# pierrebarbera/epa-ng

Hardware: AMD Instinct MI355X
Metric: query placements/sec (whole node), 512-tip GTR+G4 DNA ref, preplace+thorough (higher is better)
Workload: dtype f64; 1 GPU; cfg2: 512-tip DNA GTR+G4 ref, W=1500, 150 bp reads, dyn-heur 0.99999, preplace+thorough; branches=1021, parallelism=query-shard x1 (weak)

## Files before the change

### epa_ng_amd/csrc/epa_dev.hip

```cpp
#include "epa_dev_internal.hpp"

#include <math.h>
#include <string.h>

#include <algorithm>
#include <numeric>
#include <atomic>
#include <thread>

static thread_local std::string g_create_err;

int epa_fail(epa_ctx* ctx, int code, const std::string& msg) {
  if (ctx) ctx->err = msg; else g_create_err = msg;
  return code;
}

namespace {
__global__ void __launch_bounds__(256) k_zero(uint4* __restrict__ a, size_t na, uint4* __restrict__ b, size_t nb) {
  const size_t stride = (size_t)gridDim.x * 256, i0 = (size_t)blockIdx.x * 256 + threadIdx.x;
  const uint4 z = make_uint4(0u, 0u, 0u, 0u);
  for (size_t i = i0; i < na; i += stride) a[i] = z;
  for (size_t i = i0; i < nb; i += stride) b[i] = z;
}
}
// ... 473 lines not shown
}

double log_sum_exp(const double* v, uint32_t K) {
  double mx = v[0], sum = 0.0;
  for (uint32_t j = 1; j < K; ++j) mx = std::max(mx, v[j]);
  for (uint32_t j = 0; j < K; ++j) sum += std::exp(v[j] - mx);
  return mx + std::log(sum);
}
}

extern "C" int epa_quadrature_legendre01(uint32_t K, double* nodes, double* log_weights) {
  if (K < 1 || K > 64 || !nodes || !log_weights) return EPA_ERR_INVALID_ARG;
  std::vector<double> d(K, 0.0), o(K > 1 ? K - 1 : 0), x;
  for (uint32_t i = 1; i < K; ++i) o[i - 1] = (double)i / std::sqrt(4.0 * i * i - 1.0);
  tridiag_eigenvalues(d, o, x);
  for (uint32_t j = 0; j < K; ++j) {
    double t = x[j], dp = 1.0;
    for (int it = 0; it < 3; ++it) {
      double p0 = 1.0, p1 = t;
      for (uint32_t n = 1; n < K; ++n) { const double p2 = ((2.0 * n + 1.0) * t * p1 - n * p0) / (n + 1.0); p0 = p1; p1 = p2; }
      dp = K * (t * p1 - p0) / (t * t - 1.0);
      if (it < 2) t -= p1 / dp;
    }
    nodes[j] = 0.5 * (1.0 + t);
    log_weights[j] = -std::log((1.0 - t) * (1.0 + t)) - 2.0 * std::log(std::fabs(dp));
  }
  const double norm = log_sum_exp(log_weights, K);
  for (uint32_t j = 0; j < K; ++j) log_weights[j] -= norm;
  return EPA_OK;
}

extern "C" int epa_quadrature_laguerre(uint32_t K, double* nodes, double* log_weights) {
  if (K < 1 || K > 64 || !nodes || !log_weights) return EPA_ERR_INVALID_ARG;
  std::vector<double> d(K), o(K > 1 ? K - 1 : 0), x;
  for (uint32_t i = 0; i < K; ++i) d[i] = 2.0 * i + 1.0;
  for (uint32_t i = 1; i < K; ++i) o[i - 1] = (double)i;
  tridiag_eigenvalues(d, o, x);
  for (uint32_t j = 0; j < K; ++j) {
    double t = x[j], lm = 1.0;
    for (int it = 0; it < 3; ++it) {
      double l0 = 1.0, l1 = 1.0 - t;
      for (uint32_t n = 1; n < K; ++n) { const double l2 = ((2.0 * n + 1.0 - t) * l1 - n * l0) / (n + 1.0); l0 = l1; l1 = l2; }
      lm = l0;
      if (it < 2) t -= l1 * t / (K * (l1 - l0));
    }
    nodes[j] = t;
    log_weights[j] = std::log(t) - 2.0 * std::log((double)K) - 2.0 * std::log(std::fabs(lm));
  }
  const double norm = log_sum_exp(log_weights, K);
  for (uint32_t j = 0; j < K; ++j) log_weights[j] -= norm;
  return EPA_OK;
}

extern "C" int epa_dev_device_count(void) {
  int n = 0;
  if (hipGetDeviceCount(&n) != hipSuccess) { (void)hipGetLastError(); return 0; }
  return n;
}

extern "C" const char* epa_dev_last_error(const epa_ctx* ctx) {
  return ctx ? ctx->err.c_str() : g_create_err.c_str();
}

extern "C" int epa_dev_set_query_layout(epa_ctx* ctx, uint32_t code_stride) {
  if (!ctx) return EPA_ERR_INVALID_ARG;
  ctx->code_stride = code_stride;
  return EPA_OK;
}

extern "C" int epa_dev_set_option(epa_ctx* ctx, const char* key, int value) {
  if (!ctx || !key) return EPA_ERR_INVALID_ARG;
  if (strcmp(key, "lookup_block") == 0) {
    if (!ctx->lookup_blocks) return epa_fail(ctx, EPA_ERR_INVALID_ARG, "set_option: lookup_block needs a context in the blocked lookup layout");
    if (value <= 0 || (value & 63)) return epa_fail(ctx, EPA_ERR_INVALID_ARG, "set_option: lookup_block must be a positive multiple of 64");
    for (void* p : ctx->blk_buf)
      if (p) return epa_fail(ctx, EPA_ERR_INVALID_ARG, "set_option: lookup_block must be set before the first preplacement");
    ctx->lookup_block = (uint32_t)value;
    return EPA_OK;
  }
  const bool dedup_key = strcmp(key, "dedup_key_bits") == 0;
  if (dedup_key || strcmp(key, "dedup_sort_bits") == 0) {
    if (value < 0 || value > 64) return epa_fail(ctx, EPA_ERR_INVALID_ARG, std::string("set_option: ") + key + " must be 0 .. 64");
    (dedup_key ? ctx->opt.dedup_key_bits : ctx->opt.dedup_sort_bits) = value;
    return EPA_OK;
  }
  struct Entry { const char* name; int EpaOptions::*field; };
  static const Entry table[] = {
      {"thorough_generic", &EpaOptions::thorough_generic}, {"preplace_generic", &EpaOptions::preplace_generic},
      {"select_full_rows", &EpaOptions::select_full_rows}, {"select_sort", &EpaOptions::select_sort},
      {"queued_thorough", &EpaOptions::queued_thorough},   {"xcd_balance", &EpaOptions::xcd_balance},
      {"aa_valu", &EpaOptions::aa_valu},                   {"timers", &EpaOptions::timers},
      {"newton_lds", &EpaOptions::newton_lds},             {"tip_distal", &EpaOptions::tip_distal},
      {"preplace_screen", &EpaOptions::preplace_screen},   {"preplace_screen_scale", &EpaOptions::preplace_screen_scale}};
  for (const Entry& e : table)
    if (strcmp(key, e.name) == 0) {
      ctx->opt.*e.field = value;
      ctx->generic_thorough = ctx->generic_native || ctx->opt.thorough_generic != 0;
      return EPA_OK;
    }
  return epa_fail(ctx, EPA_ERR_INVALID_ARG, std::string("set_option: unknown key '") + key + "'");
}

extern "C" int epa_dev_set_heuristic(epa_ctx* ctx, int mode, double param) {
  if (!ctx) return EPA_ERR_INVALID_ARG;
  if (mode < EPA_HEUR_DYNAMIC || mode > EPA_HEUR_BASEBALL)
    return epa_fail(ctx, EPA_ERR_INVALID_ARG, "set_heuristic: unknown mode");
  if (mode == EPA_HEUR_FIXED && !(param >= 0.0 && param <= 1.0))
    return epa_fail(ctx, EPA_ERR_INVALID_ARG, "set_heuristic: the fraction must lie in [0, 1]");
  ctx->heur_mode = mode;
  ctx->heur_param = param;
  return EPA_OK;
}

extern "C" int epa_dev_set_query_packing(epa_ctx* ctx, int bits) {
  if (!ctx) return EPA_ERR_INVALID_ARG;
  if (bits != 8 && bits != 4) return epa_fail(ctx, EPA_ERR_INVALID_ARG, "set_query_packing: 8 or 4 bits per code");
  if (bits == 4 && ctx->s != 4)
    return epa_fail(ctx, EPA_ERR_UNSUPPORTED, "set_query_packing: the 4-bit format holds nucleotide codes only");
  ctx->code_packed4 = bits == 4;
  return EPA_OK;
}

extern "C" int epa_pack_codes_4bit(const uint8_t* codes, uint32_t Q, uint32_t stride, uint8_t* packed) {
  if (!codes || !packed) return EPA_ERR_INVALID_ARG;
  const size_t ps = ((size_t)stride + 1) / 2;
  const unsigned cap = g_encode_threads.load(std::memory_order_relaxed);
  const unsigned hw = cap ? cap : std::max(1u, std::thread::hardware_concurrency());
  const unsigned nt = (unsigned)std::min<uint64_t>(std::min(hw, 32u), std::max<uint64_t>(1, (uint64_t)Q * stride >> 20));
  std::vector<int> bad(nt, 0);
  auto work = [&](unsigned t) {
    const uint32_t q0 = (uint32_t)((uint64_t)Q * t / nt), q1 = (uint32_t)((uint64_t)Q * (t + 1) / nt);
    unsigned over = 0;
    for (uint32_t q = q0; q < q1; ++q) {
      const uint8_t* r = codes + (size_t)q * stride;
      uint8_t* o = packed + (size_t)q * ps;
      for (uint32_t p = 0; p < stride / 2; ++p) {
        const uint8_t hi = r[2 * p], lo = r[2 * p + 1];
        over |= hi | lo;
        o[p] = (uint8_t)((hi << 4) | lo);
      }
      if (stride & 1) { const uint8_t hi = r[stride - 1]; over |= hi; o[ps - 1] = (uint8_t)(hi << 4); }
    }
    bad[t] = over > 15;
  };
  if (nt == 1) work(0);
  else {
    std::vector<std::thread> th;
    for (unsigned t = 0; t < nt; ++t) th.emplace_back(work, t);
    for (auto& x : th) x.join();
  }
  for (unsigned t = 0; t < nt; ++t) if (bad[t]) return EPA_ERR_INVALID_ARG;
  return EPA_OK;
}

extern "C" int epa_unpack_codes_4bit(const uint8_t* packed, uint32_t Q, uint32_t stride, uint8_t* codes) {
  if (!codes || !packed) return EPA_ERR_INVALID_ARG;
  const size_t ps = ((size_t)stride + 1) / 2;
  for (uint32_t q = 0; q < Q; ++q)
    for (uint32_t i = 0; i < stride; ++i) {
      const uint8_t b = packed[(size_t)q * ps + i / 2];
      codes[(size_t)q * stride + i] = (i & 1) ? (b & 15u) : (b >> 4);
    }
  return EPA_OK;
}

extern "C" int epa_dev_set_stream(epa_ctx* ctx, void* s) {
// ... 1557 lines not shown
```

### epa_ng_amd/csrc/epa_dev_internal.hpp

```cpp
#pragma once

#include <hip/hip_runtime.h>
#include <stdint.h>

#include <algorithm>
#include <cmath>
#include <string>
#include <vector>

#include <rocprim/device/device_radix_sort.hpp>

#include "epa_dev.h"

using epa_radix_cfg = rocprim::radix_sort_config<rocprim::default_config, rocprim::default_config,
                                                 rocprim::default_config, 0>;

#define EPA_MAX_STATES 20
#define EPA_MAX_CATS 16
#define EPA_MAX_COLS 24
#define EPA_GRID_Y 65535u

struct ModelDNA {
  double U[16];
  double Ui[16];
// ... 135 lines not shown
  uint64_t n = 0;
  SlotState state = SlotState::Free;
  bool unfinished() const { return state == SlotState::Begun || state == SlotState::Launched || state == SlotState::GroupMember; }
  ChunkInputs staged_inputs() const {
    if (x_codes) return {x_codes, x_begin, x_span};
    const char* d = (const char*)d_in;
    const uint32_t* b = (const uint32_t*)(d + codes_bytes);
    return {(const uint8_t*)d, b, b + Q};
  }
  SelectPending sel;
  uint32_t* h_sel = nullptr;
  const uint8_t* l_codes = nullptr;
  const uint32_t *l_begin = nullptr, *l_span = nullptr;
  epa_pair* l_pairs = nullptr;
  epa_result* l_res = nullptr;
  uint32_t l_max_span = 0, l_flags = 0;
  int leader = -1;
  int g_index = 0;
  int g_n = 0;
  int g_left = 0;
  int g_slots[EPA_MAX_GROUP] = {};
  uint32_t g_qoff[EPA_MAX_GROUP + 1] = {};
  uint32_t own_Q = 0;
  const uint8_t* own_x_codes = nullptr;
  const uint32_t *own_x_begin = nullptr, *own_x_span = nullptr;
  void* d_merge = nullptr;
  size_t d_merge_sz = 0;
  epa_pair* d_gpairs = nullptr;
  epa_result* d_gres = nullptr;
  size_t g_cap = 0;
  uint32_t* d_goff = nullptr;
  uint32_t* h_goff = nullptr;

  void lead_merged(uint32_t total, const uint8_t* codes, const uint32_t* begin, const uint32_t* span) {
    own_Q = Q; own_x_codes = x_codes; own_x_begin = x_begin; own_x_span = x_span;
    Q = total; x_codes = codes; x_begin = begin; x_span = span;
  }
  void restore_own() { Q = own_Q; x_codes = own_x_codes; x_begin = own_x_begin; x_span = own_x_span; }
  void group_begun(ChunkSlot* all, const int* slots, int n, const uint32_t* qoff) {
    g_n = n;
    for (int i = 0; i <= n; ++i) g_qoff[i] = qoff[i];
    for (int i = 0; i < n; ++i) {
      g_slots[i] = slots[i];
      all[slots[i]].leader = slots[0];
      all[slots[i]].g_index = i;
      if (i) all[slots[i]].state = SlotState::GroupMember;
    }
  }
  void group_launched(ChunkSlot* all) {
    restore_own();
    g_left = g_n;
    for (int i = 1; i < g_n; ++i) {
      all[g_slots[i]].state = SlotState::Launched;
      all[g_slots[i]].l_flags = l_flags;
    }
  }
  void launch_over(ChunkSlot* all, SlotState to) {
    state = to;
    if (g_n <= 1) return;
    restore_own();
    for (int i = 0; i < g_n; ++i) {
      all[g_slots[i]].leader = -1;
      if (i) all[g_slots[i]].state = to;
    }
    g_n = 0;
    g_left = 0;
  }
};

struct EpaOptions {
  int thorough_generic = 0;
  int preplace_generic = 0;
  int select_full_rows = 0;
  int select_sort = 0;
  int queued_thorough = 0;
  int xcd_balance = 1;
  int aa_valu = 0;
  int timers = 1;
  int newton_lds = 0;
  int tip_distal = 1;
  int dedup_key_bits = 64;
  int preplace_screen = 1;
  int preplace_screen_scale = 1;
  int dedup_sort_bits = 32;
};

struct epa_ctx {
  int device = 0;
  EpaOptions opt;
  int n_cu = 256;
  hipStream_t stream = nullptr;
  std::string err;

  int s = 0, c = 0, ncols = 0;
  int c_in = 0;
  uint32_t W = 0, B = 0;
  ModelDev hmodel;
  ModelDev* dmodel = nullptr;
  ModelDNA dna;
  bool dna_zero0 = false;
  bool rate_scalers = false;
  bool generic_thorough = false;
  bool generic_native = false;
  BloConsts blo;
  int aa_x_as_n = 0;
  uint32_t code_stride = 0;

  double* refT = nullptr;
  uint32_t* scSum = nullptr;
  double* blen = nullptr;
  double* lookup = nullptr;
  double* refI = nullptr;
  uint8_t* resc0 = nullptr;
  double* cinv = nullptr;
  double inv_w0 = 0.0;
  double* lookup2 = nullptr;
  float2* lookup2f = nullptr;
  bool lookup2f_refused = false;
  uint64_t screen_runs = 0;
  double screen_M = 0.0;
  uint64_t screen_nonfinite = 0;
  uint32_t* tip_row = nullptr;
  uint8_t* tipmask = nullptr;
  double* tipd = nullptr;
  bool lookup_built = false;
  double* prof_tab = nullptr;
  bool lookup_blocks = false;
  uint32_t lookup_block = 1024;
  std::vector<double> h_blen;

  static constexpr int N_SCRATCH = 26;
  static constexpr int N_SLOTS = 24;
  static constexpr int N_BANKS = 1 + N_SLOTS;
  int bank = 0;
  void* scratch[N_BANKS * N_SCRATCH] = {};
  size_t scratch_sz[N_BANKS * N_SCRATCH] = {};

  uint32_t select_cap = 64;
  uint32_t* th_ctr = nullptr;
  bool code_packed4 = false;
  int heur_mode = 0;
  double heur_param = 0.0;

  hipStream_t copy_stream = nullptr, down_stream = nullptr;
  ChunkSlot slots[N_SLOTS];

  enum { T_PREPLACE = 0, T_THOROUGH = 1, T_SELECT = 2, T_SCORE = 3, T_SITES = 4, T_RELL = 5, T_MARGINAL = 6, T_RELL_TESTS = 7, T_RELL_AU = 8, T_RELL_KH = 9, T_PREPLACE_PROFILE = 10, T_DEDUP = 11, N_TIMERS = 12 };
  EvTimer t_lookup;
  std::vector<hipEvent_t> blk_ev[N_BANKS];
  uint32_t blk_ev_n[N_BANKS] = {};
  void* blk_buf[N_BANKS] = {};
  size_t blk_sz[N_BANKS] = {};
  EvTimer t_bank[N_BANKS][N_TIMERS];
  uint32_t xcd_cum[9] = {0u, 1u << 17, 2u << 17, 3u << 17, 4u << 17, 5u << 17, 6u << 17, 7u << 17, 1u << 20};
  double xcd_w[8] = {0.125, 0.125, 0.125, 0.125, 0.125, 0.125, 0.125, 0.125};
  double last_sclk_mhz = 0.0;
  bool xstamp_ok = false;
  hipEvent_t ev_rb[N_BANKS] = {};
  hipStream_t side_stream[N_BANKS] = {};
  hipEvent_t ev_fork[N_BANKS] = {}, ev_join[N_BANKS] = {};
  const void* clean_stats[N_BANKS] = {};
  bool clean_ctr[N_BANKS] = {};
  int t_last[N_TIMERS] = {};
  epa_thorough_stats last_stats{};
};

// ... 180 lines not shown
```

### epa_ng_amd/csrc/preplace.hip

```cpp
#include "epa_dev_internal.hpp"
#include "wave_util.hpp"

#include <cstdlib>
#include <cstring>

#include <algorithm>

namespace {

constexpr int GQ = 256;
constexpr int CH = 160;
constexpr int SPREAD = 96;
constexpr int TROWS = CH + SPREAD;
constexpr int NB = 16;
constexpr int CW = CH / 4;

struct Group {
  uint32_t start;
  uint32_t count;
  uint32_t min_begin;
  uint32_t cls;
};

__device__ __forceinline__ void validate_window(uint32_t i, uint32_t begin, uint32_t span, uint32_t W,
// ... 466 lines not shown
#define PP_XCD 1
#endif
using epa_wave::seg_key;
struct SegTrack {
  double m = -INFINITY;
  __device__ __forceinline__ void add(unsigned long long* __restrict__ segmax, uint32_t segp, uint32_t qi, uint32_t b,
                                      bool last, double v) {
    m = fmax(m, v);
    if ((b & 63u) == 63u || last) {
      atomicMax(&segmax[(size_t)qi * segp + (b >> 6)], seg_key(m));
      m = -INFINITY;
    }
  }
};

#ifndef PP_PRIO
#define PP_PRIO 1
#endif
template <int NBATCH>
__device__ __forceinline__ void gather_prio(int bt) {
#if PP_PRIO == 1
  if (bt == 0) __builtin_amdgcn_s_setprio(3);
  else if (bt == NBATCH / 4) __builtin_amdgcn_s_setprio(2);
  else if (bt == NBATCH / 2) __builtin_amdgcn_s_setprio(1);
  else if (bt == (3 * NBATCH) / 4) __builtin_amdgcn_s_setprio(0);
#elif PP_PRIO == 2
  if (bt == 0) __builtin_amdgcn_s_setprio(3);
  else if (bt == NBATCH / 2) __builtin_amdgcn_s_setprio(0);
#elif PP_PRIO == 3
  if (bt == 0) __builtin_amdgcn_s_setprio(3);
  else if (bt == (2 * NBATCH) / 5) __builtin_amdgcn_s_setprio(2);
  else if (bt == (7 * NBATCH) / 10) __builtin_amdgcn_s_setprio(1);
  else if (bt == (9 * NBATCH) / 10) __builtin_amdgcn_s_setprio(0);
#elif PP_PRIO == 4
  if (bt == 0) __builtin_amdgcn_s_setprio(3);
  else if (bt == NBATCH / 10) __builtin_amdgcn_s_setprio(2);
  else if (bt == (3 * NBATCH) / 10) __builtin_amdgcn_s_setprio(1);
  else if (bt == (6 * NBATCH) / 10) __builtin_amdgcn_s_setprio(0);
#endif
}

struct ItemWalk { uint32_t pos, end, step, lo; };
__device__ __forceinline__ ItemWalk item_walk(uint32_t total) {
  if (PP_XCD && (gridDim.x & 7u) == 0) {
    const uint32_t x = blockIdx.x & 7u, local = blockIdx.x >> 3;
    const uint32_t lo = (uint32_t)((uint64_t)total * x / 8), hi = (uint32_t)((uint64_t)total * (x + 1) / 8);
    return {lo + local, hi, gridDim.x >> 3, lo};
  }
  return {blockIdx.x, total, gridDim.x, 0u};
}

#ifndef PP_XCD_GROUPS
#define PP_XCD_GROUPS 1
#endif
__device__ __forceinline__ void item_group_tile(uint32_t v, uint32_t lo, uint32_t hi, uint32_t ng, uint32_t ntiles,
                                                uint32_t& grp, uint32_t& tile) {
  if (!PP_XCD_GROUPS) { grp = v % ng; tile = v / ng; return; }
  const uint32_t gl = lo / ntiles, tl = lo - gl * ntiles, gh = (hi - 1) / ntiles, th = (hi - 1) - gh * ntiles;
  uint32_t r = v - lo;
  for (uint32_t t = 0; t < ntiles; ++t) {
    const uint32_t first = gl + (t < tl ? 1u : 0u), last1 = gh + 1u - (t > th ? 1u : 0u);
    const uint32_t c = last1 > first ? last1 - first : 0u;
    if (r < c) { grp = first + r; tile = t; return; }
    r -= c;
  }
  grp = 0; tile = ntiles;
}

__device__ __forceinline__ uint32_t choose_tile(uint32_t ng, uint32_t B, uint32_t nwg) {
  uint32_t best = 32, best_cost = 0xffffffffu;
  for (uint32_t n = 16; n <= 96; n += 8) {
    const uint32_t items = ng * ((B + n - 1) / n);
    const uint32_t cost = ((items + nwg - 1) / nwg) * (n + 3);
    if (cost <= best_cost) { best_cost = cost; best = n; }
  }
  return best;
}

#ifdef PP_SCHED_PIN
#define PP_SCHED_BARRIER() __builtin_amdgcn_sched_barrier(0)
#else
#define PP_SCHED_BARRIER()
#endif
template <bool ACC, int SPR, int ROWL, bool SPARSE = false>
__global__ void __launch_bounds__(GQ2, 4) k_preplace_pairs(
    const double* __restrict__ lookup2, const uint16_t* __restrict__ packed,
    const uint16_t* __restrict__ tails, const uint32_t* __restrict__ win_begin,
    const uint32_t* __restrict__ win_span, const uint32_t* __restrict__ perm,
    const Group* __restrict__ groups, uint32_t W, uint32_t B, uint32_t pitch, uint32_t NP16,
    const uint32_t* __restrict__ status, double* __restrict__ lnl,
    unsigned long long* __restrict__ segmax, uint32_t segp) {
  constexpr int TR2 = (CH + SPR) / 2;
  extern __shared__ __attribute__((aligned(16))) char smem[];
  static_assert(ROWL % 16 == 0 && ROWL >= PROWB && ((TR2 - 1) * ROWL + PROWB) < 65536, "16-bit LDS offsets");
  double* accs = reinterpret_cast<double*>(smem + (size_t)TR2 * ROWL);
  __shared__ uint32_t s_maxspan;
  __shared__ uint32_t s_qi[GQ2];
  constexpr uint32_t BSTR = GQ2 + 4;
  const uint32_t ng = status[5];
  const uint32_t NBP = SPARSE ? 64u : ACC ? NB2_ACC : choose_tile(ng, B, gridDim.x);
  const uint32_t ntiles = SPARSE ? 1u : (B + NBP - 1) / NBP;
  const int t = threadIdx.x;
  const ItemWalk iw = SPARSE ? ItemWalk{blockIdx.x, ng, gridDim.x, 0u} : item_walk(ng * ntiles);
  for (uint32_t item = iw.pos; item < iw.end; item += iw.step) {
  uint32_t item_g = item, item_t = 0;
  if (!SPARSE) item_group_tile(item, iw.lo, iw.end, ng, ntiles, item_g, item_t);
  const Group g = groups[item_g];
  const uint32_t b0 = SPARSE ? min(g.min_begin * 64u, B - 1u) : item_t * NBP;
  const uint32_t nb = min(NBP, B - b0);
  __syncthreads();
  if (g.count == 0) continue;
  const bool active = t < (int)g.count;
  uint32_t qi = 0, begin = 0, span = 0;
  if (active) {
    qi = perm[g.start + t];
    begin = win_begin[qi];
    span = win_span[qi];
    if ((uint64_t)begin + span > W) span = 0;
  }
  if (t == 0) s_maxspan = 0;
  const uint32_t my_q = (active && span > 0) ? qi : 0xffffffffu;
  s_qi[t] = my_q;
  __syncthreads();
  {
    uint32_t m = span;
#pragma unroll
    for (int off = 32; off; off >>= 1) m = max(m, (uint32_t)__shfl_xor((int)m, off));
    if ((t & 63) == 0) atomicMax(&s_maxspan, m);
  }
  if (ACC) for (uint32_t j = 0; j < nb; ++j) accs[j * GQ2 + t] = 0.0;
  __syncthreads();
  const uint32_t gmin = win_begin[perm[g.start]];
  const uint32_t gspread = win_begin[perm[g.start + g.count - 1]] - gmin;
  const uint32_t rowoff = ((begin - gmin) >> 1) * ROWL;
  const uint32_t rowoff2 = rowoff | (rowoff << 16);
  const uint32_t nchunks = ACC ? (s_maxspan + CH - 1) / CH : 1;
  uint32_t t0 = 0, t1 = 0, t2 = 0, tailchunk = 0xffffffffu;
  if (active && (span & 3)) {
    const uint16_t* tq = tails + (size_t)qi * 4;
    t0 = tq[0] + rowoff; t1 = tq[1] + rowoff; t2 = tq[2] + rowoff;
    tailchunk = ((span >> 2) * 2) / CP;
  }
  auto at = [&](uint32_t off) -> double { return *reinterpret_cast<const double*>(smem + off); };
  SegTrack seg;

  for (uint32_t c = 0; c < nchunks; ++c) {
    const uint32_t cbase = c * CH;
    const bool mine = active && cbase < span;
    uint32_t cw[PW];
    if (mine) {
      const uint4* p = reinterpret_cast<const uint4*>(packed + (size_t)qi * NP16 + (size_t)c * CP);
#pragma unroll
      for (int i = 0; i < PW / 4; ++i) {
        const uint4 v = p[i];
        cw[4 * i] = v.x + rowoff2;
        cw[4 * i + 1] = v.y + rowoff2;
        cw[4 * i + 2] = v.z + rowoff2;
        cw[4 * i + 3] = v.w + rowoff2;
      }
    } else {
#pragma unroll
      for (int i = 0; i < PW; ++i) cw[i] = 0;
    }
    const uint32_t row0 = gmin + cbase;
    const uint32_t need = min((uint32_t)TR2, (gspread >> 1) + (min((uint32_t)CH, s_maxspan - cbase) + 1) / 2);
    const uint32_t rows = (row0 < W) ? min(need, (W - row0 + 1) / 2) : 0;
    const uint32_t n2 = rows * (PE / 2);
    constexpr int PF = (TR2 * (PE / 2) + GQ2 - 1) / GQ2;
    auto request = [&](uint32_t j, double2 (&pfs)[PF]) {
      const double2* src = reinterpret_cast<const double2*>(
          lookup2 + (((size_t)(b0 + j) * 2 + (row0 & 1u)) * ((W + 1) / 2) + (row0 >> 1)) * PE);
#pragma unroll
      for (int u = 0; u < PF; ++u) {
        const uint32_t i = u * GQ2 + t;
        pfs[u] = make_double2(0.0, 0.0);
        if (i < n2) pfs[u] = src[i];
      }
    };
    auto stage = [&](const double2 (&pfs)[PF], uint32_t boff) {
#pragma unroll
      for (int u = 0; u < PF; ++u) {
        const uint32_t i = u * GQ2 + t;
        if (i < n2) {
          if (ROWL == PROWB) {
            reinterpret_cast<double2*>(smem + boff)[i] = pfs[u];
          } else {
            const uint32_t r = i / (PE / 2), c2 = i - r * (PE / 2);
            *reinterpret_cast<double2*>(smem + boff + r * ROWL + c2 * 16) = pfs[u];
          }
        }
      }
    };
    auto gather = [&](uint32_t j, uint32_t boff) {
      if (mine) {
        double sum = ACC ? accs[j * GQ2 + t] : 0.0;
#pragma unroll
        for (int i = 0; i < PW; ++i) asm volatile("" : "+v"(cw[i]));
#ifndef PP_WPB
#define PP_WPB 2
#endif
        constexpr int WPB = PP_WPB, NBATCH = PW / WPB;
        double rb[2][WPB * 2];
        auto issue = [&](int bt) {
#pragma unroll
          for (int w = 0; w < WPB; ++w) {
            const uint32_t v = cw[bt * WPB + w];
            rb[bt & 1][2 * w] = at((v & 0xffffu) + boff);
            rb[bt & 1][2 * w + 1] = at((v >> 16) + boff);
          }
        };
        issue(0);
        PP_SCHED_BARRIER();
#pragma unroll
        for (int bt = 0; bt < NBATCH; ++bt) {
          gather_prio<NBATCH>(bt);
          if (bt + 1 < NBATCH) issue(bt + 1);
          PP_SCHED_BARRIER();
#pragma unroll
          for (int w = 0; w < WPB; ++w) {
            const double s1 = rb[bt & 1][2 * w] + rb[bt & 1][2 * w + 1];
            sum += s1;
          }
          PP_SCHED_BARRIER();
        }
        if (c == tailchunk) {
          sum += at(t0 + boff);
          sum += at(t1 + boff);
          sum += at(t2 + boff);
        }
        if (ACC) {
          accs[j * GQ2 + t] = sum;
        } else {
          accs[(j & 7u) * BSTR + t] = sum;
          if (segmax) seg.add(segmax, segp, qi, b0 + j, j + 1 == nb, sum);
        }
      }
    };
    auto emit_burst = [&](uint32_t kb) {
      __builtin_amdgcn_wave_barrier();
      const uint32_t lane = (uint32_t)t & 63u, wbase = (uint32_t)t & ~63u, c4 = lane & 3u;
      const uint32_t ncol = min(8u, nb - 8u * kb), bcol = b0 + 8u * kb + 2u * c4;
      const uint32_t r0 = 2u * c4, r1 = 2u * c4 + 1u;
#pragma unroll
      for (uint32_t k = 0; k < 4; ++k) {
        const uint32_t tq = wbase + k * 16 + (lane >> 2);
        const uint32_t q = s_qi[tq];
        if (q != 0xffffffffu && 2u * c4 < ncol) {
          const double a0 = accs[r0 * BSTR + tq];
          double* dst = lnl + (size_t)q * pitch + bcol;
          if (2u * c4 + 1u < ncol) *reinterpret_cast<double2*>(dst) = make_double2(a0, accs[r1 * BSTR + tq]);
          else *dst = a0;
        }
      }
      __builtin_amdgcn_wave_barrier();
    };
    auto flush = [&](uint32_t j) {
      if (ACC) return;
      if ((j & 7u) == 7u) emit_burst(j >> 3);
      else if (j + 1 == nb) emit_burst(j >> 3);
    };
    {
      double2 pf[PF];
      request(0, pf);
      for (uint32_t j = 0; j < nb; ++j) {
        __syncthreads();
        stage(pf, 0);
        __syncthreads();
        if (j + 1 < nb) request(j + 1, pf);
        PP_SCHED_BARRIER();
        gather(j, 0);
        flush(j);
// ... 548 lines not shown
  const uint32_t K = pairs ? n_blocks * Wp : sites ? ctx->W + 1 : 0;
  size_t temp_bytes = 0;
  (void)rocprim::radix_sort_pairs<epa_radix_cfg>(nullptr, temp_bytes, (uint32_t*)nullptr, (uint32_t*)nullptr,
                                  (uint32_t*)nullptr, (uint32_t*)nullptr, Q, 0, 32, ctx->stream);
  uint32_t *status, *key_cnt, *iota, *sorted_keys, *perm, *keys;
  const uint32_t nseg = (ctx->B + 63) / 64, seg32p = (nseg + 7u) & ~7u;
  const uint32_t KB = 2 * Wp, n_blocks_c = 2 * nseg;
  const uint64_t max_cells = (uint64_t)Q * nseg;
  const uint32_t Kc = nseg * KB + 1;
  const uint32_t max_runs_c = (uint32_t)std::min<uint64_t>((max_cells + GQ2 - 1) / GQ2 + n_blocks_c, 0xffffffu);
  const uint32_t max_groups_c = max_runs_c + n_blocks_c * n_buckets;
  const size_t smem_c = sizeof(uint32_t) * (2 * (n_blocks_c + 1) + 4 * (size_t)max_runs_c + 2);
  double delta = -1.0;
  constexpr uint64_t SCREEN_MIN_CELLS = 80000000ull;
  const bool big = ctx->opt.preplace_screen >= 2 || probe || (uint64_t)Q * ctx->B >= SCREEN_MIN_CELLS;
  if (pairs && !blocked && nseg <= 64 && max_span != 0 && max_span <= (uint32_t)CH && ctx->opt.preplace_screen && big &&
      (probe || (segmax && t.band_t > 0.0)) && max_cells < 0x80000000ull && smem_c <= 65536) {
    const int brc = launch_build_lookup2f(ctx);
    if (brc) return brc;
    delta = epa_screen_delta(ctx, span_bound);
  }
  const bool screen = delta >= 0.0;
  uint32_t *seg32, *cstatus, *ccnt, *crank, *csorted, *cperm;
  unsigned long long *seg_mask, *n_incl;
  Group* cgroups;
  Group* groups;
  uint16_t *packed, *tails;
  void* temp;
  auto layout = [&](Carver c) {
    status = c.take<uint32_t>(64);
    key_cnt = c.take<uint32_t>(K);
    seg32 = c.take<uint32_t>(screen ? (size_t)Q * seg32p : 0);
    n_incl = c.take<unsigned long long>(screen ? 1 : 0);
    cstatus = c.take<uint32_t>(screen ? 64 : 0);
    ccnt = c.take<uint32_t>(screen ? Kc : 0);
    iota = c.take<uint32_t>(Q);
    sorted_keys = c.take<uint32_t>(Q);
    perm = c.take<uint32_t>(Q);
    keys = c.take<uint32_t>(Q);
    groups = c.take<Group>(max_groups);
    packed = c.take<uint16_t>((size_t)Q * NP16);
    tails = c.take<uint16_t>((pairs || sites) ? 4 * (size_t)Q : 0);
    seg_mask = c.take<unsigned long long>(screen ? Q : 0);
    crank = c.take<uint32_t>(screen ? (size_t)Q * seg32p : 0);
    csorted = c.take<uint32_t>(screen ? max_cells : 0);
    cperm = c.take<uint32_t>(screen ? max_cells : 0);
    cgroups = c.take<Group>(screen ? max_groups_c : 0);
    temp = c.tail(temp_bytes);
    return c.off;
  };
  char* base = (char*)epa_scratch(ctx, SLOT_PREPLACE, layout(Carver{}));
  if (!base) return epa_fail(ctx, EPA_ERR_HIP, "hipMalloc(preplace scratch)");
  layout(Carver{base});
  *d_status = status;
  {
    const int zr = epa_zero_async(ctx, status, (char*)iota - (char*)status, segmax, sizeof(unsigned long long) * (size_t)Q * segp);
    if (zr) return zr;
  }
  const bool acc = max_span == 0 || max_span > (uint32_t)CH;
  const bool wide = pairs && !acc && (uint64_t)Q * SPREAD < (uint64_t)1400 * ctx->W;
  const uint32_t rowl = (wide || acc) ? ROWL_PACKED : ROWL_NARROW;
  if (pairs) {
    constexpr uint32_t pack_grid = 64;
    hipLaunchKernelGGL(k_pack_pairs, dim3(std::min<uint32_t>((Q + 15) / 16, (uint32_t)ctx->n_cu * pack_grid)), dim3(256), 0, ctx->stream, d_codes, d_begin,
                       d_span, Q, ctx->W, cstride, crel, span_bound, Wp, NP16, rowl, packed, tails, keys, K, status);
  } else if (sites) {
    hipLaunchKernelGGL(k_pack_sites<24>, dim3((Q + 3) / 4), dim3(256), 0, ctx->stream, d_codes, d_begin,
                       d_span, Q, ctx->W, cstride, crel, span_bound, NP16, packed, tails, keys, K, status);
  }
  if (pairs || sites) {
    hipLaunchKernelGGL(k_count_keys, dim3((Q + 255) / 256), dim3(256), 0, ctx->stream, keys, Q, key_cnt, iota);
    launch_scan_counts(ctx, key_cnt, K);
    hipLaunchKernelGGL(k_scatter_sorted, dim3((Q + 255) / 256), dim3(256), 0, ctx->stream, keys, iota, key_cnt, Q,
                       sorted_keys, perm);
  } else {
    hipLaunchKernelGGL(k_iota, dim3((Q + 255) / 256), dim3(256), 0, ctx->stream, iota, Q);
    hipLaunchKernelGGL(k_validate, dim3((Q + 255) / 256), dim3(256), 0, ctx->stream, d_begin, d_span, Q,
                       ctx->W, std::min(span_bound, crel ? cstride : 0xffffffffu), status);
    int wbits = 1;
    while (wbits < 32 && (1ull << wbits) <= (uint64_t)ctx->W) ++wbits;
    EPA_HIP(ctx, rocprim::radix_sort_pairs<epa_radix_cfg>(temp, temp_bytes, d_begin, sorted_keys, iota, perm, Q, 0, wbits,
                                           ctx->stream));
  }
  constexpr int SPREAD_WIDE = 288;
  hipLaunchKernelGGL(k_make_groups, dim3(1), dim3(256),
                     sizeof(uint32_t) * (2 * (n_blocks + 1) + 4 * (size_t)max_runs + 2), ctx->stream,
                     sorted_keys, Q, pairs ? Wp : 0xffffffffu, n_blocks, class_blocks, gq0, gq1,
                     (uint32_t)(wide ? SPREAD_WIDE : SPREAD), max_runs, groups, max_groups, status);
  const size_t codes_bytes = (size_t)Q * cstride;
  const uint32_t want_cls = pairs ? 1u : 0u;
  const size_t lds = sizeof(double) * ((size_t)TROWS * ctx->ncols + (acc ? (size_t)NB * GQ : 0));
  const size_t lds2 = wide ? (size_t)((CH + SPREAD_WIDE) / 2) * ROWL_PACKED + sizeof(double) * NB2_BURST * (GQ2 + 4)
                           : (size_t)TROWS2 * rowl + sizeof(double) * (acc ? NB2_ACC * GQ2 : NB2_BURST * (GQ2 + 4));
  const bool acc_s = max_span == 0 || max_span > (uint32_t)CHS;
  const size_t lds_s = (size_t)TROWS_S * 24 * 8 + sizeof(double) * (acc_s ? NB2_ACC_S * GQ2 : NB2_BURST * (GQ2 + 4));
  using FastKernel = decltype(&k_preplace_sites<24, false>);
  using GenericKernel = decltype(&k_preplace<16, false>);
  FastKernel k_fast = nullptr;
  if (pairs) k_fast = wide ? k_preplace_pairs<false, SPREAD_WIDE, ROWL_PACKED> : acc ? k_preplace_pairs<true, SPREAD, ROWL_PACKED> : k_preplace_pairs<false, SPREAD, ROWL_NARROW>;
  else if (sites) k_fast = acc_s ? k_preplace_sites<24, true> : k_preplace_sites<24, false>;
  const bool fast_acc = pairs ? acc : acc_s;
  const size_t lds_fast = pairs ? lds2 : lds_s;
  const GenericKernel k_generic = sites ? nullptr : ctx->ncols == 16 ? (acc ? k_preplace<16, true> : k_preplace<16, false>) : (acc ? k_preplace<24, true> : k_preplace<24, false>);
  if (k_fast) EPA_HIP(ctx, hipFuncSetAttribute((const void*)k_fast, hipFuncAttributeMaxDynamicSharedMemorySize, (int)lds_fast));
  if (k_generic) EPA_HIP(ctx, hipFuncSetAttribute((const void*)k_generic, hipFuncAttributeMaxDynamicSharedMemorySize, (int)lds));
  auto kernels = [&](const double* lk, const double* lk2, uint32_t nB, double* lnl, unsigned long long* sm, bool fast = true) {
    if (k_fast && fast) {
      const uint32_t tile = fast_acc ? (pairs ? NB2_ACC : NB2_ACC_S) : 16;
      const dim3 grid_f((uint32_t)std::min<uint64_t>((uint64_t)max_groups * ((nB + tile - 1) / tile), (uint64_t)ctx->n_cu));
      hipLaunchKernelGGL(k_fast, grid_f, dim3(GQ2), (uint32_t)lds_fast, ctx->stream, pairs ? lk2 : lk, (const uint16_t*)packed,
                         (const uint16_t*)tails, d_begin, d_span, perm, groups, ctx->W, nB, pitch, NP16, status, lnl,
                         fast_acc ? nullptr : sm, segp);
    }
    if (!k_generic) return;
    const uint32_t ntiles = (nB + NB - 1) / NB;
    const dim3 grid(pairs ? (uint32_t)std::min<uint64_t>((uint64_t)max_groups * ntiles, (uint64_t)ctx->n_cu * (acc ? 2 : 4))
                          : max_groups * ntiles);
    hipLaunchKernelGGL(k_generic, grid, dim3(GQ), (uint32_t)lds, ctx->stream, lk, d_codes, d_begin, d_span, perm, groups, ctx->W,
                       cstride, crel, nB, pitch, codes_bytes, want_cls, status, lnl);
  };
  if (probe) probe->ran = screen;
  if (probe && !screen) return EPA_OK;
  if (screen) {
    using ScreenKernel = decltype(&k_preplace_screen<SPREAD, ROWL_NARROW>);
    const ScreenKernel k_screen = wide ? k_preplace_screen<SPREAD_WIDE, ROWL_PACKED> : k_preplace_screen<SPREAD, ROWL_NARROW>;
    const FastKernel k_exact = wide ? k_preplace_pairs<false, SPREAD_WIDE, ROWL_PACKED, true> : k_preplace_pairs<false, SPREAD, ROWL_NARROW, true>;
    const size_t lds_scr = wide ? (size_t)((CH + SPREAD_WIDE) / 2) * ROWL_PACKED : (size_t)TROWS2 * ROWL_NARROW;
    EPA_HIP(ctx, hipFuncSetAttribute((const void*)k_screen, hipFuncAttributeMaxDynamicSharedMemorySize, (int)lds_scr));
    EPA_HIP(ctx, hipFuncSetAttribute((const void*)k_exact, hipFuncAttributeMaxDynamicSharedMemorySize, (int)lds_fast));
    const uint32_t BP = (ctx->B + 1) / 2;
    struct Events {
      hipEvent_t e[3] = {nullptr, nullptr, nullptr};
      ~Events() { for (hipEvent_t x : e) if (x) (void)hipEventDestroy(x); }
    } evs;
    hipEvent_t* const ev = evs.e;
    if (probe) for (hipEvent_t& e : evs.e) EPA_HIP(ctx, hipEventCreate(&e));
    if (probe) EPA_HIP(ctx, hipEventRecord(ev[0], ctx->stream));
    else epa_timer_start(ctx, epa_t(ctx, epa_ctx::T_PREPLACE));
    const dim3 grid_s((uint32_t)std::min<uint64_t>((uint64_t)max_groups * ((BP + 15) / 16), (uint64_t)ctx->n_cu));
    hipLaunchKernelGGL(k_screen, grid_s, dim3(GQ2), (uint32_t)lds_scr, ctx->stream, (const float2*)ctx->lookup2f, (const uint16_t*)packed,
                       (const uint16_t*)tails, d_begin, d_span, perm, groups, ctx->W, BP, NP16, status, seg32, seg32p);
    if (probe) EPA_HIP(ctx, hipEventRecord(ev[1], ctx->stream));
    const double band = (probe ? probe->band_t : t.band_t) + 2.0 * delta;
    hipLaunchKernelGGL(k_screen_band, dim3((Q + 255) / 256), dim3(256), 0, ctx->stream, (const uint32_t*)seg32, Q, nseg, seg32p, band,
                       delta, (const uint32_t*)keys, KB, probe ? nullptr : segmax, segp, probe ? nullptr : ccnt, crank, seg_mask, n_incl);
    if (probe) {
      EPA_HIP(ctx, hipEventRecord(ev[2], ctx->stream));
      EPA_HIP(ctx, hipGetLastError());
      EPA_HIP(ctx, hipEventSynchronize(ev[2]));
      (void)hipEventElapsedTime(&probe->ms_screen, ev[0], ev[1]);
      (void)hipEventElapsedTime(&probe->ms_band, ev[1], ev[2]);
      probe->delta = delta;
      probe->seg32 = seg32;
      probe->mask = seg_mask;
      probe->n_incl = n_incl;
      return EPA_OK;
    }
    ++ctx->screen_runs;
    launch_scan_counts(ctx, ccnt, Kc);
    hipLaunchKernelGGL(k_scatter_cells, dim3((Q + 255) / 256), dim3(256), 0, ctx->stream, (const unsigned long long*)seg_mask,
                       (const uint32_t*)keys, (const uint32_t*)crank, (const uint32_t*)ccnt, Q, seg32p, KB, (uint32_t)max_cells, csorted, cperm);
    hipLaunchKernelGGL(k_make_groups, dim3(1), dim3(256), smem_c, ctx->stream, (const uint32_t*)csorted, (uint32_t)max_cells, Wp, n_blocks_c,
                       n_blocks_c, (uint32_t)GQ2, (uint32_t)GQ2, (uint32_t)(wide ? SPREAD_WIDE : SPREAD), max_runs_c, cgroups, max_groups_c,
                       cstatus, (const uint32_t*)(ccnt + (Kc - 1)), KB);
    hipLaunchKernelGGL(k_exact, dim3(std::min<uint32_t>(max_groups_c, (uint32_t)ctx->n_cu)), dim3(GQ2), (uint32_t)lds_fast, ctx->stream,
                       (const double*)ctx->lookup2, (const uint16_t*)packed, (const uint16_t*)tails, d_begin, d_span, (const uint32_t*)cperm,
                       (const Group*)cgroups, ctx->W, ctx->B, pitch, NP16, (const uint32_t*)cstatus, d_lnl, segmax, segp);
    kernels(ctx->lookup, ctx->lookup2, ctx->B, d_lnl, segmax, false);
    epa_timer_stop(ctx, epa_t(ctx, epa_ctx::T_PREPLACE));
    EPA_HIP(ctx, hipGetLastError());
    return EPA_OK;
  }
  if (!blocked) {
    epa_timer_start(ctx, epa_t(ctx, epa_ctx::T_PREPLACE));
    kernels(ctx->lookup, ctx->lookup2, ctx->B, d_lnl, segmax);
    epa_timer_stop(ctx, epa_t(ctx, epa_ctx::T_PREPLACE));
    EPA_HIP(ctx, hipGetLastError());
    return EPA_OK;
  }
  const uint32_t blk = epa_block_branches(ctx);
  size_t off2 = 0;
  (void)epa_block_bytes(ctx->s, ctx->W, blk, &off2);
  char* buf = (char*)epa_block_buffer(ctx);
  if (!buf) return epa_fail(ctx, EPA_ERR_NO_MEMORY, "hipMalloc(lookup block buffer): " + std::to_string(epa_block_bytes(ctx->s, ctx->W, blk, nullptr)) +
                                                    " bytes needed for blocks of " + std::to_string(blk) + " branches (option lookup_block)");
  double* blk_lookup = reinterpret_cast<double*>(buf);
  double* blk_lookup2 = ctx->s == 4 ? reinterpret_cast<double*>(buf + off2) : nullptr;
  const uint32_t nblocks = (ctx->B + blk - 1) / blk;
  std::vector<hipEvent_t>& ev = ctx->blk_ev[ctx->bank];
  const bool timed = ctx->opt.timers != 0;
  ctx->blk_ev_n[ctx->bank] = 0;
  (void)epa_t(ctx, epa_ctx::T_PREPLACE);
  auto mark = [&](uint32_t i) -> int {
    if (!timed) return EPA_OK;
    while (ev.size() <= i) { hipEvent_t e = nullptr; EPA_HIP(ctx, hipEventCreate(&e)); ev.push_back(e); }
    EPA_HIP(ctx, hipEventRecord(ev[i], ctx->stream));
    return EPA_OK;
  };
  for (uint32_t k = 0; k < nblocks; ++k) {
    const uint32_t b0 = k * blk, nB = std::min(blk, ctx->B - b0);
    int rc = mark(2 * k);
    if (!rc) rc = launch_build_lookup_block(ctx, b0, nB, blk_lookup);
    if (!rc && pairs) rc = launch_build_lookup2_block(ctx, nB, blk_lookup, blk_lookup2);
    if (!rc) rc = mark(2 * k + 1);
    if (rc) return rc;
    kernels(blk_lookup, blk_lookup2, nB, d_lnl + b0, segmax ? segmax + (b0 >> 6) : nullptr);
  }
  { const int rc = mark(2 * nblocks); if (rc) return rc; }
  if (timed) ctx->blk_ev_n[ctx->bank] = 2 * nblocks + 1;
  EPA_HIP(ctx, hipGetLastError());
  return EPA_OK;
}

int preplace_window_error(epa_ctx* ctx, const uint32_t* st) {
  if (st[0])
    return epa_fail(ctx, EPA_ERR_QUERY_ALL_GAP, "Sequence " + std::to_string(st[0] & 0x7fffffffu) +
                                                    " does not appear to have any non-gap sites!");
  if (st[1])
    return epa_fail(ctx, EPA_ERR_QUERY_WIDTH, "Query sequence length not same as reference alignment!");
  return EPA_OK;
}

int preplace_check_status(epa_ctx* ctx, const uint32_t* d_status) {
  uint32_t st[4];
  EPA_HIP(ctx, hipMemcpy(st, d_status, sizeof(st), hipMemcpyDeviceToHost));
  return preplace_window_error(ctx, st);
}
```

Measured before the change: 17.99 million placements/s.

## Split exact preplace pass into branch sub-tiles and always group with wide spread

The exact (sparse) preplace kernel now splits each group's 64-branch cell into sub-tiles of 8 to 64 branches. The tile size comes from a cost model or a new exact_tile option, and the launch grid grows to up to eight times the group count so more workgroups share the work. Groups for the exact pass are always built with the wide spread. When the narrow row layout is in use, packed offsets are converted on the fly with a magic-number division so the wide slice can be staged. This aims to fix load imbalance when few groups survive screening, at the cost of repeated per-tile setup and extra offset arithmetic.

```diff
diff --git a/epa_ng_amd/csrc/epa_dev.hip b/epa_ng_amd/csrc/epa_dev.hip
--- a/epa_ng_amd/csrc/epa_dev.hip
+++ b/epa_ng_amd/csrc/epa_dev.hip
@@ -579,6 +579,12 @@
   if (dedup_key || strcmp(key, "dedup_sort_bits") == 0) {
     if (value < 0 || value > 64) return epa_fail(ctx, EPA_ERR_INVALID_ARG, std::string("set_option: ") + key + " must be 0 .. 64");
     (dedup_key ? ctx->opt.dedup_key_bits : ctx->opt.dedup_sort_bits) = value;
+    return EPA_OK;
+  }
+  if (strcmp(key, "exact_tile") == 0) {
+    if (value != 0 && value != 8 && value != 16 && value != 32 && value != 64)
+      return epa_fail(ctx, EPA_ERR_INVALID_ARG, "set_option: exact_tile must be 0, 8, 16, 32 or 64");
+    ctx->opt.exact_tile = value;
     return EPA_OK;
   }
   struct Entry { const char* name; int EpaOptions::*field; };
diff --git a/epa_ng_amd/csrc/epa_dev_internal.hpp b/epa_ng_amd/csrc/epa_dev_internal.hpp
--- a/epa_ng_amd/csrc/epa_dev_internal.hpp
+++ b/epa_ng_amd/csrc/epa_dev_internal.hpp
@@ -241,6 +241,7 @@
   int dedup_key_bits = 64;
   int preplace_screen = 1;
   int preplace_screen_scale = 1;
+  int exact_tile = 0;
   int dedup_sort_bits = 32;
 };
 
diff --git a/epa_ng_amd/csrc/preplace.hip b/epa_ng_amd/csrc/preplace.hip
--- a/epa_ng_amd/csrc/preplace.hip
+++ b/epa_ng_amd/csrc/preplace.hip
@@ -572,6 +572,23 @@
 #else
 #define PP_SCHED_BARRIER()
 #endif
+constexpr int SPREAD_WIDE = 288;
+constexpr uint32_t EXACT_SETUP = 5;
+constexpr uint32_t DIV384_MAGIC = 11184811u;
+__device__ __forceinline__ uint32_t exact_offset(uint32_t o) { return o - 96u * __umulhi(o, DIV384_MAGIC); }
+__device__ __forceinline__ uint32_t exact_offset2(uint32_t w) {
+  return exact_offset(w & 0xffffu) | (exact_offset(w >> 16) << 16);
+}
+__device__ __forceinline__ uint32_t choose_exact_tile(uint32_t ng, uint32_t nwg) {
+  uint32_t best = 64, best_cost = 0xffffffffu;
+  for (uint32_t n = 8; n <= 64; n <<= 1) {
+    const uint32_t items = ng * (64u / n);
+    const uint32_t cost = ((items + nwg - 1) / nwg) * (n + EXACT_SETUP);
+    if (cost <= best_cost) { best_cost = cost; best = n; }
+  }
+  return best;
+}
+
 template <bool ACC, int SPR, int ROWL, bool SPARSE = false>
 __global__ void __launch_bounds__(GQ2, 4) k_preplace_pairs(
     const double* __restrict__ lookup2, const uint16_t* __restrict__ packed,
@@ -581,25 +598,31 @@
     const uint32_t* __restrict__ status, double* __restrict__ lnl,
     unsigned long long* __restrict__ segmax, uint32_t segp) {
   constexpr int TR2 = (CH + SPR) / 2;
+  constexpr int LROWL = SPARSE ? ROWL_PACKED : ROWL;
+  constexpr bool CONVERT = SPARSE && ROWL == ROWL_NARROW;
+  static_assert(!SPARSE || (SPR == SPREAD_WIDE && !ACC && (ROWL == ROWL_NARROW || ROWL == ROWL_PACKED)), "the exact pass stages the wide slice");
   extern __shared__ __attribute__((aligned(16))) char smem[];
-  static_assert(ROWL % 16 == 0 && ROWL >= PROWB && ((TR2 - 1) * ROWL + PROWB) < 65536, "16-bit LDS offsets");
-  double* accs = reinterpret_cast<double*>(smem + (size_t)TR2 * ROWL);
+  static_assert(LROWL % 16 == 0 && LROWL >= PROWB && ((TR2 - 1) * LROWL + PROWB) < 65536, "16-bit LDS offsets");
+  double* accs = reinterpret_cast<double*>(smem + (size_t)TR2 * LROWL);
   __shared__ uint32_t s_maxspan;
   __shared__ uint32_t s_qi[GQ2];
   constexpr uint32_t BSTR = GQ2 + 4;
   const uint32_t ng = status[5];
-  const uint32_t NBP = SPARSE ? 64u : ACC ? NB2_ACC : choose_tile(ng, B, gridDim.x);
-  const uint32_t ntiles = SPARSE ? 1u : (B + NBP - 1) / NBP;
+  const uint32_t forced = SPARSE ? status[6] : 0u;
+  const uint32_t NBP = SPARSE ? (forced ? forced : choose_exact_tile(ng, gridDim.x))
+                              : ACC ? NB2_ACC : choose_tile(ng, B, gridDim.x);
+  const uint32_t ntiles = SPARSE ? 64u / NBP : (B + NBP - 1) / NBP;
   const int t = threadIdx.x;
-  const ItemWalk iw = SPARSE ? ItemWalk{blockIdx.x, ng, gridDim.x, 0u} : item_walk(ng * ntiles);
+  const ItemWalk iw = SPARSE ? ItemWalk{blockIdx.x, ng * ntiles, gridDim.x, 0u} : item_walk(ng * ntiles);
   for (uint32_t item = iw.pos; item < iw.end; item += iw.step) {
-  uint32_t item_g = item, item_t = 0;
-  if (!SPARSE) item_group_tile(item, iw.lo, iw.end, ng, ntiles, item_g, item_t);
+  uint32_t item_g, item_t;
+  if (SPARSE) { item_g = item % ng; item_t = item / ng; }
+  else item_group_tile(item, iw.lo, iw.end, ng, ntiles, item_g, item_t);
   const Group g = groups[item_g];
-  const uint32_t b0 = SPARSE ? min(g.min_begin * 64u, B - 1u) : item_t * NBP;
-  const uint32_t nb = min(NBP, B - b0);
+  const uint32_t b0 = (SPARSE ? g.min_begin * 64u : 0u) + item_t * NBP;
+  const uint32_t nb = (SPARSE && b0 >= B) ? 0u : min(NBP, B - b0);
   __syncthreads();
-  if (g.count == 0) continue;
+  if (g.count == 0 || (SPARSE && nb == 0)) continue;
   const bool active = t < (int)g.count;
   uint32_t qi = 0, begin = 0, span = 0;
   if (active) {
@@ -622,13 +645,15 @@
   __syncthreads();
   const uint32_t gmin = win_begin[perm[g.start]];
   const uint32_t gspread = win_begin[perm[g.start + g.count - 1]] - gmin;
-  const uint32_t rowoff = ((begin - gmin) >> 1) * ROWL;
+  const uint32_t rowoff = ((begin - gmin) >> 1) * LROWL;
   const uint32_t rowoff2 = rowoff | (rowoff << 16);
   const uint32_t nchunks = ACC ? (s_maxspan + CH - 1) / CH : 1;
   uint32_t t0 = 0, t1 = 0, t2 = 0, tailchunk = 0xffffffffu;
   if (active && (span & 3)) {
     const uint16_t* tq = tails + (size_t)qi * 4;
-    t0 = tq[0] + rowoff; t1 = tq[1] + rowoff; t2 = tq[2] + rowoff;
+    t0 = tq[0]; t1 = tq[1]; t2 = tq[2];
+    if (CONVERT) { t0 = exact_offset(t0); t1 = exact_offset(t1); t2 = exact_offset(t2); }
+    t0 += rowoff; t1 += rowoff; t2 += rowoff;
     tailchunk = ((span >> 2) * 2) / CP;
   }
   auto at = [&](uint32_t off) -> double { return *reinterpret_cast<const double*>(smem + off); };
@@ -642,7 +667,8 @@
       const uint4* p = reinterpret_cast<const uint4*>(packed + (size_t)qi * NP16 + (size_t)c * CP);
 #pragma unroll
       for (int i = 0; i < PW / 4; ++i) {
-        const uint4 v = p[i];
+        uint4 v = p[i];
+        if (CONVERT) v = make_uint4(exact_offset2(v.x), exact_offset2(v.y), exact_offset2(v.z), exact_offset2(v.w));
         cw[4 * i] = v.x + rowoff2;
         cw[4 * i + 1] = v.y + rowoff2;
         cw[4 * i + 2] = v.z + rowoff2;
@@ -672,11 +698,11 @@
       for (int u = 0; u < PF; ++u) {
         const uint32_t i = u * GQ2 + t;
         if (i < n2) {
-          if (ROWL == PROWB) {
+          if (LROWL == PROWB) {
             reinterpret_cast<double2*>(smem + boff)[i] = pfs[u];
           } else {
             const uint32_t r = i / (PE / 2), c2 = i - r * (PE / 2);
-            *reinterpret_cast<double2*>(smem + boff + r * ROWL + c2 * 16) = pfs[u];
+            *reinterpret_cast<double2*>(smem + boff + r * LROWL + c2 * 16) = pfs[u];
           }
         }
       }
@@ -1391,7 +1417,6 @@
     EPA_HIP(ctx, rocprim::radix_sort_pairs<epa_radix_cfg>(temp, temp_bytes, d_begin, sorted_keys, iota, perm, Q, 0, wbits,
                                            ctx->stream));
   }
-  constexpr int SPREAD_WIDE = 288;
   hipLaunchKernelGGL(k_make_groups, dim3(1), dim3(256),
                      sizeof(uint32_t) * (2 * (n_blocks + 1) + 4 * (size_t)max_runs + 2), ctx->stream,
                      sorted_keys, Q, pairs ? Wp : 0xffffffffu, n_blocks, class_blocks, gq0, gq1,
@@ -1433,10 +1458,12 @@
   if (screen) {
     using ScreenKernel = decltype(&k_preplace_screen<SPREAD, ROWL_NARROW>);
     const ScreenKernel k_screen = wide ? k_preplace_screen<SPREAD_WIDE, ROWL_PACKED> : k_preplace_screen<SPREAD, ROWL_NARROW>;
-    const FastKernel k_exact = wide ? k_preplace_pairs<false, SPREAD_WIDE, ROWL_PACKED, true> : k_preplace_pairs<false, SPREAD, ROWL_NARROW, true>;
+    const FastKernel k_exact = rowl == (uint32_t)ROWL_NARROW ? k_preplace_pairs<false, SPREAD_WIDE, ROWL_NARROW, true>
+                                                              : k_preplace_pairs<false, SPREAD_WIDE, ROWL_PACKED, true>;
     const size_t lds_scr = wide ? (size_t)((CH + SPREAD_WIDE) / 2) * ROWL_PACKED : (size_t)TROWS2 * ROWL_NARROW;
+    const size_t lds_exact = (size_t)((CH + SPREAD_WIDE) / 2) * ROWL_PACKED + sizeof(double) * NB2_BURST * (GQ2 + 4);
     EPA_HIP(ctx, hipFuncSetAttribute((const void*)k_screen, hipFuncAttributeMaxDynamicSharedMemorySize, (int)lds_scr));
-    EPA_HIP(ctx, hipFuncSetAttribute((const void*)k_exact, hipFuncAttributeMaxDynamicSharedMemorySize, (int)lds_fast));
+    EPA_HIP(ctx, hipFuncSetAttribute((const void*)k_exact, hipFuncAttributeMaxDynamicSharedMemorySize, (int)lds_exact));
     const uint32_t BP = (ctx->B + 1) / 2;
     struct Events {
       hipEvent_t e[3] = {nullptr, nullptr, nullptr};
@@ -1470,11 +1497,13 @@
     hipLaunchKernelGGL(k_scatter_cells, dim3((Q + 255) / 256), dim3(256), 0, ctx->stream, (const unsigned long long*)seg_mask,
                        (const uint32_t*)keys, (const uint32_t*)crank, (const uint32_t*)ccnt, Q, seg32p, KB, (uint32_t)max_cells, csorted, cperm);
     hipLaunchKernelGGL(k_make_groups, dim3(1), dim3(256), smem_c, ctx->stream, (const uint32_t*)csorted, (uint32_t)max_cells, Wp, n_blocks_c,
-                       n_blocks_c, (uint32_t)GQ2, (uint32_t)GQ2, (uint32_t)(wide ? SPREAD_WIDE : SPREAD), max_runs_c, cgroups, max_groups_c,
+                       n_blocks_c, (uint32_t)GQ2, (uint32_t)GQ2, (uint32_t)SPREAD_WIDE, max_runs_c, cgroups, max_groups_c,
                        cstatus, (const uint32_t*)(ccnt + (Kc - 1)), KB);
-    hipLaunchKernelGGL(k_exact, dim3(std::min<uint32_t>(max_groups_c, (uint32_t)ctx->n_cu)), dim3(GQ2), (uint32_t)lds_fast, ctx->stream,
-                       (const double*)ctx->lookup2, (const uint16_t*)packed, (const uint16_t*)tails, d_begin, d_span, (const uint32_t*)cperm,
-                       (const Group*)cgroups, ctx->W, ctx->B, pitch, NP16, (const uint32_t*)cstatus, d_lnl, segmax, segp);
+    if (ctx->opt.exact_tile) EPA_HIP(ctx, hipMemsetD32Async(reinterpret_cast<hipDeviceptr_t>(cstatus + 6), ctx->opt.exact_tile, 1, ctx->stream));
+    hipLaunchKernelGGL(k_exact, dim3((uint32_t)std::min<uint64_t>((uint64_t)max_groups_c * 8, (uint64_t)ctx->n_cu)), dim3(GQ2),
+                       (uint32_t)lds_exact, ctx->stream, (const double*)ctx->lookup2, (const uint16_t*)packed, (const uint16_t*)tails, d_begin,
+                       d_span, (const uint32_t*)cperm, (const Group*)cgroups, ctx->W, ctx->B, pitch, NP16, (const uint32_t*)cstatus, d_lnl,
+                       segmax, segp);
     kernels(ctx->lookup, ctx->lookup2, ctx->B, d_lnl, segmax, false);
     epa_timer_stop(ctx, epa_t(ctx, epa_ctx::T_PREPLACE));
     EPA_HIP(ctx, hipGetLastError());
```

Result: no change. 18.17 million placements/s, median of 6 (+1.0%).
